# avi22bhattacharya/ThinkDiff-mlre

Hardware: AMD Instinct MI355X
Metric: images/sec (1024², 28 steps) ThinkDiff-CLIP FLUX.1 at 1/2/4/8 MI355X (higher is better)
Workload: dtype bf16

## Files before the change

thinkdiff-mlre_amd/csrc/attention_bf16.hip:

```cpp
#include "attention_common.h"

template <bool CAUSAL, int NWAVES, bool BIAS = false, bool VARLEN = false, bool PRE = false, bool RS = true, bool FIXED = false>
__global__ __launch_bounds__(NWAVES * 64, 2) void td_attn_fwd_d128_lean_kernel(const TdAttnParams p) {
#if defined(__HIP_DEVICE_COMPILE__)
  extern __shared__ __attribute__((aligned(16))) char smem[];

  const int tid = threadIdx.x;
  const int lane = tid & 63;
  const int wid = __builtin_amdgcn_readfirstlane(tid >> 6);
  const int h5 = lane >> 5;
  const int l31 = lane & 31;

  const int qblk = blockIdx.x;
  const int head = blockIdx.y;
  const int batch = blockIdx.z;
  const int kvhead = head / p.q_per_kv;
  const int q0 = qblk * (NWAVES * Q_WAVE) + wid * Q_WAVE;

  const bf16_t* Qb = p.Q + (size_t)batch * p.q_bstride;
  const bf16_t* Kb = p.K + (size_t)batch * p.kv_bstride;
  const bf16_t* Vb = p.V + (size_t)batch * p.kv_bstride;
  bf16_t* Ob = p.O + (size_t)batch * p.o_bstride;
  int Sq = p.Sq, Skv = p.Skv, c_off = p.causal_offset;
  if constexpr (VARLEN) {
// ... 276 lines not shown

      f32x16_t st[2];
      attn_tile_scores<PO, FIXED>(st, qf, kone, qnegm, ka);

      const int key0 = t * KV_TILE;
      if (key0 + KV_TILE > Skv) {
#pragma unroll
        for (int kk = 0; kk < 2; ++kk)
#pragma unroll
          for (int rr = 0; rr < 16; ++rr) {
            const int key = key0 + kk * 32 + (rr & 3) + 8 * (rr >> 2) + 4 * h5;
            if (key >= Skv) st[kk][rr] = -INFINITY;
          }
      }

      attn_tile_softmax_pv<PO, PRE, RS, FIXED>(st, o, lacc, m_run, qnegm, t == kb, c, va, h5);
    };
    {
      int t = kb;
      for (; t + 1 < ke; t += 2) {
        tile(t, std::integral_constant<unsigned, 0>{});
        tile(t + 1, std::integral_constant<unsigned, 1>{});
      }
      if (t < ke) tile(t, std::integral_constant<unsigned, 0>{});
    }
    float l_run = RS ? lacc[0] : half_swap_sum(lacc[0]);
    if (kb > 0 || ke < nt) {
      const int j = kb > 0 ? r : r + 1;
      const bool tail = kb > 0;
      const __amdgpu_buffer_rsrc_t rsS = __builtin_amdgcn_make_buffer_rsrc((void*)(ws + SK_HEADER_BYTES), 0, (unsigned)(2 * G) * SK_SLOT_FLOATS * 4u, 0x00020000);
      const unsigned lane_off = ((unsigned)wid * 17u * 64u + (unsigned)lane) * 16u;
      const unsigned mine = (unsigned)(tail ? j : G + j) * (SK_SLOT_FLOATS * 4u) + lane_off;
      const unsigned theirs = (unsigned)(tail ? G + j : j) * (SK_SLOT_FLOATS * 4u) + lane_off;
      auto ask = [&](bool draw) -> unsigned {
        __syncthreads();
        if (tid == 0)
          *ticket_lds = draw ? __hip_atomic_fetch_add(cnt + j, 1u, __ATOMIC_RELAXED, __HIP_MEMORY_SCOPE_AGENT)
                             : __hip_atomic_load(cnt + j, __ATOMIC_RELAXED, __HIP_MEMORY_SCOPE_AGENT);
        __syncthreads();
        return *ticket_lds;
      };
      bool other_ready = !tail && ask(false) == 1u;
      if (!other_ready) {
#pragma unroll
        for (int q4 = 0; q4 < 16; ++q4) {
          const u32x4_t v = {as_u32(o[q4 >> 2][4 * (q4 & 3)]), as_u32(o[q4 >> 2][4 * (q4 & 3) + 1]),
                             as_u32(o[q4 >> 2][4 * (q4 & 3) + 2]), as_u32(o[q4 >> 2][4 * (q4 & 3) + 3])};
          __builtin_amdgcn_raw_buffer_store_b128(v, rsS, mine + q4 * 1024u, 0, 16);
        }
        const u32x4_t ml = {as_u32(m_run), as_u32(l_run), 0u, 0u};
        __builtin_amdgcn_raw_buffer_store_b128(ml, rsS, mine + 16 * 1024u, 0, 16);
        asm volatile("s_waitcnt vmcnt(0)" ::: "memory");
        other_ready = ask(true) == 1u;
        if (!other_ready) continue;
      }
      if (tid == 0) __builtin_amdgcn_fence(__ATOMIC_ACQUIRE, "agent");
      asm volatile("s_waitcnt vmcnt(0)" ::: "memory");
      __syncthreads();
      const u32x4_t ml = __builtin_amdgcn_raw_buffer_load_b128(rsS, theirs + 16 * 1024u, 0, 0);
      const float m2 = as_f32(ml[0]), l2 = as_f32(ml[1]);
      const float mm = fmaxf(m_run, m2);
      const float a1 = __builtin_amdgcn_exp2f((m_run - mm) * cc), a2 = __builtin_amdgcn_exp2f((m2 - mm) * cc);
      auto comb = [&](float own, float other) {
        return tail ? __builtin_fmaf(other, a2, own * a1) : __builtin_fmaf(own, a1, other * a2);
      };
      l_run = comb(l_run, l2);
#pragma unroll
      for (int q4 = 0; q4 < 16; ++q4) {
        const u32x4_t v = __builtin_amdgcn_raw_buffer_load_b128(rsS, theirs + q4 * 1024u, 0, 0);
#pragma unroll
        for (int k4 = 0; k4 < 4; ++k4)
          o[q4 >> 2][4 * (q4 & 3) + k4] = comb(o[q4 >> 2][4 * (q4 & 3) + k4], as_f32(v[k4]));
      }
      if (tid == 0) __hip_atomic_store(cnt + j, 0u, __ATOMIC_RELAXED, __HIP_MEMORY_SCOPE_AGENT);
    }

    const float inv = 1.0f / l_run;
    const int q = q0 + l31;
    if (p.q8) {
      const int qr = min(q, p.Sq - 1);
      attn_store_rows_q8(o, inv, p.q8 + (size_t)qr * p.ldq8 + head * D, h5, p.q8_inv[qr], p.q8_amax + qr, q < p.Sq);
    } else {
      attn_store_rows(o, inv, p.O + (size_t)batch * p.o_bstride + (size_t)min(q, p.Sq - 1) * p.ldo + head * D, h5, (p.ldo & 7) == 0 && !(p.variant & 0x200), q < p.Sq);
    }
  }
#endif
}

namespace {

size_t sk_ws_bytes(int ranges) { return (size_t)SK_HEADER_BYTES + (size_t)2 * ranges * SK_SLOT_FLOATS * sizeof(float); }

int sk_pooled_workspace(int dev, int ranges, hipStream_t stream, char** out) {
  struct Entry { int dev; hipStream_t stream; int ranges; char* ws; };
  static std::mutex mu;
  static std::vector<Entry> pool;
  std::lock_guard<std::mutex> lock(mu);
  for (auto& e : pool)
    if (e.dev == dev && e.stream == stream && e.ranges >= ranges) { *out = e.ws; return 0; }
  char* w = nullptr;
  TD_CHECK_HIP(hipMalloc((void**)&w, sk_ws_bytes(ranges)));
  TD_CHECK_HIP(hipMemsetAsync(w, 0, SK_HEADER_BYTES, stream));
  pool.push_back(Entry{dev, stream, ranges, w});
  *out = w;
  return 0;
}

int device_cus(int dev) {
  static std::atomic<int> cus[64] = {};
  int n = cus[dev & 63].load(std::memory_order_relaxed);
  if (n == 0) {
    hipDeviceProp_t prop;
    if (hipGetDeviceProperties(&prop, dev) != hipSuccess) return 0;
    n = prop.multiProcessorCount;
    cus[dev & 63].store(n, std::memory_order_relaxed);
  }
  return n;
}

template <typename K>
int set_lds_attr_once(K kernel, int bytes, std::atomic<unsigned long long>& done, int dev) {
  if (!((done.load(std::memory_order_acquire) >> (dev & 63)) & 1ull)) {
    TD_CHECK_HIP(hipFuncSetAttribute((const void*)kernel, hipFuncAttributeMaxDynamicSharedMemorySize, bytes));
    done.fetch_or(1ull << (dev & 63), std::memory_order_release);
  }
  return 0;
}

}

int td_attn_device_cus(int dev) { return device_cus(dev); }
int td_attn_pooled_workspace(int dev, int ranges, hipStream_t stream, char** out) { return sk_pooled_workspace(dev, ranges, stream, out); }
int td_attn_set_lds_attr(const void* kernel, int bytes, std::atomic<unsigned long long>& done, int dev) {
  if (!((done.load(std::memory_order_acquire) >> (dev & 63)) & 1ull)) {
    TD_CHECK_HIP(hipFuncSetAttribute(kernel, hipFuncAttributeMaxDynamicSharedMemorySize, bytes));
    done.fetch_or(1ull << (dev & 63), std::memory_order_release);
  }
  return 0;
}

int td_attn_launch(const TdAttnParams& p, hipStream_t stream) {
  TD_CHECK_ARG(p.head_dim == D, "td_attention: head_dim=%d unsupported (only 128)", p.head_dim);
  TD_CHECK_ARG(p.Sq > 0 && p.Skv > 0 && p.Hq > 0 && p.Hkv > 0 && p.batch > 0, "td_attention: empty problem");
  TD_CHECK_ARG(p.Hq % p.Hkv == 0, "td_attention: Hq=%d not a multiple of Hkv=%d", p.Hq, p.Hkv);
  TD_CHECK_ARG(p.ldq % 8 == 0 && p.ldkv % 8 == 0 && p.ldo % 4 == 0, "td_attention: row strides must be 16-byte multiples");
  TD_CHECK_ARG(((long long)(p.Sq + 256) * p.ldq) * 2 < (1ll << 32) && ((long long)(p.Skv + 64) * p.ldkv) * 2 < (1ll << 32),
               "td_attention: per-batch operand exceeds the 4 GiB buffer-descriptor range");
  TD_CHECK_ARG(((uintptr_t)p.Q | (uintptr_t)p.K | (uintptr_t)p.V | (uintptr_t)p.O) % 16 == 0, "td_attention: pointers must be 16-byte aligned");
  if (p.Sq == 1 && p.causal && !p.bias && (p.variant & 0xff) == 0 && (p.kv_lens || p.causal_offset == p.Skv - 1))
    return td_attn_decode_launch(p, stream);
  TdAttnParams q = p;
  q.q_per_kv = p.Hq / p.Hkv;
  constexpr int NW = 8;
  constexpr int lds = 4 * TILE_BYTES;
  int dev = 0;
  TD_CHECK_HIP(hipGetDevice(&dev));
  static std::atomic<unsigned long long> a0{0}, a1{0}, a2{0}, a3{0}, a4{0}, a5{0};
  dim3 grid((p.Sq + NW * Q_WAVE - 1) / (NW * Q_WAVE), p.Hq, p.batch);
  if (p.bias) TD_CHECK_ARG(p.Skv % 4 == 0 && ((uintptr_t)p.bias) % 16 == 0 && p.batch == 1, "td_attention: bias needs Skv %% 4 == 0, 16-byte alignment, batch 1");
  if (p.kv_lens) TD_CHECK_ARG(p.causal && !p.bias, "td_attention: per-sequence kv lengths exist for the causal kernel only");
  if (p.q_prescaled) TD_CHECK_ARG(!p.causal && !p.bias && !p.kv_lens && !p.seg_starts, "td_attention: pre-scaled q is a form of the joint (unmasked) attention only");
  TD_CHECK_ARG(p.score_bound >= 0.f && p.score_bound <= 48.f && (p.score_bound == 0.f || p.q_prescaled), "td_attention: a score bound goes with pre-scaled q (joint attention) and lies in (0, 48] octaves (0 = none)");
  if (p.q8) TD_CHECK_ARG(!p.causal && !p.bias && !p.kv_lens && !p.seg_starts && p.batch == 1 && p.q8_inv && p.q8_amax && p.ldq8 % 8 == 0 && ((uintptr_t)p.q8) % 8 == 0,
                         "td_attention: the int8 output form is for the joint attention of one batch entry, with 8-byte aligned rows");
  if (p.seg_starts) {
    TD_CHECK_ARG(!p.bias && !p.kv_lens && p.Sq == p.Skv && (!p.causal || p.causal_offset == 0),
                 "td_attention(varlen): full or causal (offset 0) attention inside each segment only (no bias or cache lengths)");
    if (p.causal) {
      static std::atomic<unsigned long long> a12{0};
      if (int e = set_lds_attr_once(td_attn_fwd_d128_lean_kernel<true, NW, false, true>, lds, a12, dev)) return e;
      hipLaunchKernelGGL((td_attn_fwd_d128_lean_kernel<true, NW, false, true>), grid, dim3(NW * 64), lds, stream, q);
      TD_CHECK_LAUNCH();
      return 0;
    }
    static std::atomic<unsigned long long> a6{0};
    if (int e = set_lds_attr_once(td_attn_fwd_d128_lean_kernel<false, NW, false, true>, lds, a6, dev)) return e;
    hipLaunchKernelGGL((td_attn_fwd_d128_lean_kernel<false, NW, false, true>), grid, dim3(NW * 64), lds, stream, q);
    TD_CHECK_LAUNCH();
    return 0;
  }

  const int n_items = (int)(grid.x * grid.y * grid.z);
  const int cus = device_cus(dev);
  const int nt = (p.Skv + KV_TILE - 1) / KV_TILE;
  if (!p.causal && !p.bias && !p.kv_lens && (p.variant & 0xff) != 1 && cus > 0 && n_items > cus && cus < SK_MAX_RANGES && (long long)n_items * nt < (1ll << 31)) {
    char* ws = (char*)p.sk_ws;
    if (!ws) {
      if (int rc = sk_pooled_workspace(dev, cus, stream, &ws)) return rc;
    }
    constexpr int lds_sk = lds + 16;
    if (p.q_prescaled && p.score_bound > 0.f) {
      static std::atomic<unsigned long long> a10{0};
      if (int e = set_lds_attr_once(td_attn_fwd_d128_streamk_kernel<NW, true, true, true, true>, lds_sk, a10, dev)) return e;
      hipLaunchKernelGGL((td_attn_fwd_d128_streamk_kernel<NW, true, true, true, true>), dim3(cus), dim3(NW * 64), lds_sk, stream, q, ws, (int)grid.x, nt);
    } else if (p.q_prescaled) {
      static std::atomic<unsigned long long> a7{0};
      if (int e = set_lds_attr_once(td_attn_fwd_d128_streamk_kernel<NW, true, true>, lds_sk, a7, dev)) return e;
      hipLaunchKernelGGL((td_attn_fwd_d128_streamk_kernel<NW, true, true>), dim3(cus), dim3(NW * 64), lds_sk, stream, q, ws, (int)grid.x, nt);
    } else if ((p.variant & 0xff) == 2) {
      if (int e = set_lds_attr_once(td_attn_fwd_d128_streamk_kernel<NW, false>, lds_sk, a4, dev)) return e;
      hipLaunchKernelGGL((td_attn_fwd_d128_streamk_kernel<NW, false>), dim3(cus), dim3(NW * 64), lds_sk, stream, q, ws, (int)grid.x, nt);
    } else {
      if (int e = set_lds_attr_once(td_attn_fwd_d128_streamk_kernel<NW, true>, lds_sk, a5, dev)) return e;
      hipLaunchKernelGGL((td_attn_fwd_d128_streamk_kernel<NW, true>), dim3(cus), dim3(NW * 64), lds_sk, stream, q, ws, (int)grid.x, nt);
    }
    TD_CHECK_LAUNCH();
    return 0;
  }
  if (p.bias) {
    if (p.causal) {
      if (int e = set_lds_attr_once(td_attn_fwd_d128_lean_kernel<true, NW, true>, lds, a0, dev)) return e;
      hipLaunchKernelGGL((td_attn_fwd_d128_lean_kernel<true, NW, true>), grid, dim3(NW * 64), lds, stream, q);
    } else {
      if (int e = set_lds_attr_once(td_attn_fwd_d128_lean_kernel<false, NW, true>, lds, a1, dev)) return e;
      hipLaunchKernelGGL((td_attn_fwd_d128_lean_kernel<false, NW, true>), grid, dim3(NW * 64), lds, stream, q);
    }
  } else {
    if (p.q_prescaled && p.score_bound > 0.f) {
      static std::atomic<unsigned long long> a11{0};
      if (int e = set_lds_attr_once(td_attn_fwd_d128_lean_kernel<false, NW, false, false, true, true, true>, lds, a11, dev)) return e;
      hipLaunchKernelGGL((td_attn_fwd_d128_lean_kernel<false, NW, false, false, true, true, true>), grid, dim3(NW * 64), lds, stream, q);
    } else if (p.q_prescaled) {
      static std::atomic<unsigned long long> a8{0};
      if (int e = set_lds_attr_once(td_attn_fwd_d128_lean_kernel<false, NW, false, false, true>, lds, a8, dev)) return e;
      hipLaunchKernelGGL((td_attn_fwd_d128_lean_kernel<false, NW, false, false, true>), grid, dim3(NW * 64), lds, stream, q);
    } else if (p.causal) {
      if (int e = set_lds_attr_once(td_attn_fwd_d128_lean_kernel<true, NW>, lds, a2, dev)) return e;
      hipLaunchKernelGGL((td_attn_fwd_d128_lean_kernel<true, NW>), grid, dim3(NW * 64), lds, stream, q);
    } else {
      if (int e = set_lds_attr_once(td_attn_fwd_d128_lean_kernel<false, NW>, lds, a3, dev)) return e;
      hipLaunchKernelGGL((td_attn_fwd_d128_lean_kernel<false, NW>), grid, dim3(NW * 64), lds, stream, q);
    }
  }
  TD_CHECK_LAUNCH();
  return 0;
}

size_t td_attn_streamk_ws_bytes() {
  int dev = 0;
  if (hipGetDevice(&dev) != hipSuccess) return 0;
  const int cus = device_cus(dev);
  return cus > 0 && cus < SK_MAX_RANGES ? sk_ws_bytes(cus) : 0;
}
```

thinkdiff-mlre_amd/csrc/attention_common.h:

```cpp
#pragma once
#include <atomic>
#include <mutex>
#include <type_traits>
#include <vector>

#include "td_common.h"
#include "td_kernels.h"

namespace {

constexpr int D = 128;
constexpr int KV_TILE = 64;
constexpr int Q_WAVE = 32;
constexpr int TILE_BYTES = KV_TILE * D * 2;

__device__ __forceinline__ void half_swap(float x, float& lo, float& hi) {
  lo = x;
  hi = x;
  asm volatile("s_nop 1\n\tv_permlane32_swap_b32 %0, %1\n\ts_nop 1" : "+v"(lo), "+v"(hi));
}
__device__ __forceinline__ float max3(float a, float b, float c) {
  float r;
  asm("v_max3_f32 %0, %1, %2, %3" : "=v"(r) : "v"(a), "v"(b), "v"(c));
  return r;
// ... 104 lines not shown
      }
      pf[kb][s] = __builtin_bit_cast(bf16x8_t, pk);
    }
  }
  if constexpr (!RS) lacc[0] += psum;

  constexpr int VPF = 2;
  const bf16x8_t ones8 = {0x3F80, 0x3F80, 0x3F80, 0x3F80, 0x3F80, 0x3F80, 0x3F80, 0x3F80};
  bf16x4_t v0[16], v1[16];
  attn_static_for<VPF>([&](auto ec) {
    constexpr int e = decltype(ec)::value;
    v0[e] = attn_ds_read_tr16<PO + (e >> 2) * 16 * 256>(va[0][e & 3]);
    v1[e] = attn_ds_read_tr16<PO + (e >> 2) * 16 * 256>(va[1][e & 3]);
  });
  attn_static_for<16>([&](auto ec) {
    constexpr int e = decltype(ec)::value;
    if constexpr (e + VPF < 16) {
      v0[e + VPF] = attn_ds_read_tr16<PO + ((e + VPF) >> 2) * 16 * 256>(va[0][(e + VPF) & 3]);
      v1[e + VPF] = attn_ds_read_tr16<PO + ((e + VPF) >> 2) * 16 * 256>(va[1][(e + VPF) & 3]);
    }
    constexpr int behind = 2 * (15 - e < VPF ? 15 - e : VPF);
    asm volatile("s_waitcnt lgkmcnt(%2)" : "+v"(v0[e]), "+v"(v1[e]) : "n"(behind));
    bf16x8_t vf;
    vf[0] = v0[e][0]; vf[1] = v0[e][1]; vf[2] = v0[e][2]; vf[3] = v0[e][3];
    vf[4] = v1[e][0]; vf[5] = v1[e][1]; vf[6] = v1[e][2]; vf[7] = v1[e][3];
    o[e & 3] = __builtin_amdgcn_mfma_f32_32x32x16_bf16(vf, pf[e >> 3][(e >> 2) & 1], o[e & 3], 0, 0, 0);
    if constexpr (RS && (e & 3) == 3) lacc = __builtin_amdgcn_mfma_f32_32x32x16_bf16(ones8, pf[e >> 3][(e >> 2) & 1], lacc, 0, 0, 0);
    __builtin_amdgcn_sched_barrier(0x006);
  });
}

__device__ __forceinline__ void attn_store_rows(const f32x16_t (&o)[4], const float inv, bf16_t* row_ptr, const int h5, const bool wide, const bool live) {
  if (wide) {
#pragma unroll
    for (int db = 0; db < 4; ++db)
#pragma unroll
      for (int g = 0; g < 4; g += 2) {
        unsigned a0 = pack_bf2(o[db][4 * g] * inv, o[db][4 * g + 1] * inv), a1 = pack_bf2(o[db][4 * g + 2] * inv, o[db][4 * g + 3] * inv);
        unsigned b0 = pack_bf2(o[db][4 * g + 4] * inv, o[db][4 * g + 5] * inv), b1 = pack_bf2(o[db][4 * g + 6] * inv, o[db][4 * g + 7] * inv);
        const auto r0 = __builtin_amdgcn_permlane32_swap(a0, b0, false, false);
        const auto r1 = __builtin_amdgcn_permlane32_swap(a1, b1, false, false);
        const u32x4_t w = {r0[0], r1[0], r0[1], r1[1]};
        if (live) *(u32x4_t*)(row_ptr + db * 32 + 8 * (g + h5)) = w;
      }
  } else {
#pragma unroll
    for (int db = 0; db < 4; ++db)
#pragma unroll
      for (int g = 0; g < 4; ++g) {
        u32x2_t w;
        w[0] = pack_bf2(o[db][4 * g] * inv, o[db][4 * g + 1] * inv);
        w[1] = pack_bf2(o[db][4 * g + 2] * inv, o[db][4 * g + 3] * inv);
        if (live) *(u32x2_t*)(row_ptr + 4 * h5 + db * 32 + 8 * g) = w;
      }
  }
}

__device__ __forceinline__ void attn_store_rows_q8(const f32x16_t (&o)[4], const float inv, uint8_t* row_ptr, const int h5, const float qinv, unsigned* amax,
                                                   const bool live) {
  float am = 0.f;
#pragma unroll
  for (int db = 0; db < 4; ++db)
#pragma unroll
    for (int g = 0; g < 4; g += 2) {
      unsigned w[2];
#pragma unroll
      for (int h = 0; h < 2; ++h) {
        unsigned acc = 0;
#pragma unroll
        for (int b = 0; b < 4; ++b) {
          const float v = rbf(o[db][4 * (g + h) + b] * inv);
          am = fmaxf(am, fabsf(v));
          acc |= ((unsigned)__float2int_rn(fminf(fmaxf(v * qinv, -127.f), 127.f)) & 0xffu) << (8 * b);
        }
        w[h] = acc;
      }
      const auto r = __builtin_amdgcn_permlane32_swap(w[0], w[1], false, false);
      if (live) *(u32x2_t*)(row_ptr + db * 32 + 8 * (g + h5)) = u32x2_t{r[0], r[1]};
    }
  am = half_swap_max(am);
  if (live && h5 == 0) __hip_atomic_fetch_max(amax, as_u32(am), __ATOMIC_RELAXED, __HIP_MEMORY_SCOPE_AGENT);
}

}

int td_attn_set_lds_attr(const void* kernel, int bytes, std::atomic<unsigned long long>& done, int dev);

namespace {
constexpr int SK_SLOT_FLOATS = 8 * 64 * 68;
constexpr int SK_HEADER_BYTES = 4096;
constexpr int SK_MAX_RANGES = SK_HEADER_BYTES / 4 - 16;
}
```

thinkdiff-mlre_amd/csrc/capi.hip:

```cpp
#include <cstdarg>
#include <cstdio>
#include "td_kernels.h"
#include "../../include/thinkdiff_hip.h"

static thread_local char g_err[512] = "";

void td_set_error(const char* fmt, ...) {
  va_list ap;
  va_start(ap, fmt);
  vsnprintf(g_err, sizeof(g_err), fmt, ap);
  va_end(ap);
}

extern "C" {

const char* td_last_error(void) { return g_err; }
int td_abi_version(void) { return 1; }

int td_linear_bf16(const void* x, int64_t ldx, const void* w, const void* bias, void* y, int64_t ldy,
                   int M, int N, int K, int act, const void* gate, const void* res, int64_t ldr,
                   void* stream) {
  TdGemmParams p;
  p.A = (const bf16_t*)x; p.lda = (int)ldx;
  p.W = (const bf16_t*)w; p.bias = (const bf16_t*)bias;
// ... 3 lines not shown
  return td_gemm_launch(p, (hipStream_t)stream);
}

int td_linear_split_bf16(const void* x, int64_t ldx, const void* w, const void* bias,
                         void* y0, int64_t ldy0, int act0, void* y1, int64_t ldy1, int act1,
                         int M, int N, int K, int n_split, void* stream) {
  TdGemmParams p;
  p.A = (const bf16_t*)x; p.lda = (int)ldx;
  p.W = (const bf16_t*)w; p.bias = (const bf16_t*)bias;
  p.C = (bf16_t*)y0; p.ldc = (int)ldy0; p.act = act0;
  p.C2 = (bf16_t*)y1; p.ldc2 = (int)ldy1; p.act2 = act1; p.n_split = n_split;
  p.M = M; p.N = N; p.K = K;
  return td_gemm_launch(p, (hipStream_t)stream);
}

int td_linear_splitk_bf16(const void* x, int64_t ldx, const void* w, const void* bias, void* y0, int64_t ldy0, void* y1, int64_t ldy1, int n_split,
                          int M, int N, int K, const void* res, int64_t ldr, int tile_cfg, int split_k,
                          const void* norm_w, void* norm_out, int64_t ld_norm, float norm_eps, void* stream) {
  TdGemmParams p;
  p.sk_norm_w = (const bf16_t*)norm_w; p.sk_norm_out = (bf16_t*)norm_out; p.sk_norm_ld = (int)ld_norm; p.sk_norm_eps = norm_eps;
  p.A = (const bf16_t*)x; p.lda = (int)ldx; p.W = (const bf16_t*)w; p.bias = (const bf16_t*)bias;
  p.C = (bf16_t*)y0; p.ldc = (int)ldy0; p.C2 = (bf16_t*)y1; p.ldc2 = (int)ldy1; p.n_split = y1 ? n_split : 0;
  p.res = (const bf16_t*)res; p.ldr = (int)ldr; p.M = M; p.N = N; p.K = K; p.cfg = tile_cfg; p.split_k = split_k;
  return td_gemm_launch(p, (hipStream_t)stream);
}

int td_linear_grouped2_bf16(const void* x0, int M0, const void* w0, const void* bias0, const void* gate0,
                            const void* res0, void* y0, const void* x1, int M1, const void* w1,
                            const void* bias1, const void* gate1, const void* res1, void* y1,
                            int64_t ldx, int64_t ldy, int64_t ldr, int N, int K, int act, int tile_cfg,
                            void* stream) {
  TdGemmParams p;
  p.A = (const bf16_t*)x0; p.W = (const bf16_t*)w0; p.bias = (const bf16_t*)bias0; p.gate = (const bf16_t*)gate0;
  p.res = (const bf16_t*)res0; p.C = (bf16_t*)y0; p.M = M0;
  p.g_A = (const bf16_t*)x1; p.g_W = (const bf16_t*)w1; p.g_bias = (const bf16_t*)bias1; p.g_gate = (const bf16_t*)gate1;
  p.g_res = (const bf16_t*)res1; p.g_C = (bf16_t*)y1; p.g_M = M1;
  p.lda = (int)ldx; p.ldc = (int)ldy; p.ldr = (int)ldr; p.N = N; p.K = K; p.act = act; p.cfg = tile_cfg;
  return td_gemm_launch(p, (hipStream_t)stream);
}

int td_conv3x3_nhwc_bf16(const void* x, const void* w, const void* bias, const void* res, void* y,
                         int H, int W, int Cin, int Cout, int upsample2x, void* stream) {
  TdGemmParams p;
  p.A = (const bf16_t*)x; p.lda = Cin; p.W = (const bf16_t*)w; p.bias = (const bf16_t*)bias;
  p.C = (bf16_t*)y; p.ldc = Cout; p.res = (const bf16_t*)res; p.ldr = Cout;
  p.M = H * W; p.N = Cout; p.K = 9 * Cin;
  p.conv_H = H; p.conv_W = W; p.conv_Cin = Cin; p.conv_up = upsample2x ? 1 : 0;
  return td_gemm_launch(p, (hipStream_t)stream);
}

int td_linear_f32out_bf16(const void* x, int64_t ldx, const void* w, const void* bias, float* y, int64_t ldy,
                          int M, int N, int K, void* stream) {
  TdGemmParams p;
  p.A = (const bf16_t*)x; p.lda = (int)ldx; p.W = (const bf16_t*)w; p.bias = (const bf16_t*)bias;
  p.C = (bf16_t*)y; p.ldc = (int)ldy; p.M = M; p.N = N; p.K = K; p.out_f32 = 1; p.cfg = (N <= 64) ? 1 : (M <= 32 ? 2 : 0);
  return td_gemm_launch(p, (hipStream_t)stream);
}

static int g_attn_variant = 0;
int td_attention_set_variant(int variant) {
  const int prev = g_attn_variant;
  g_attn_variant = variant;
  return prev;
}

int td_attention_bf16(const void* q, int64_t ldq, int64_t q_bstride, const void* k, const void* v,
                      int64_t ldkv, int64_t kv_bstride, void* o, int64_t ldo, int64_t o_bstride,
                      int batch, int Sq, int Skv, int Hq, int Hkv, int head_dim, float scale,
                      int causal, void* stream) {
  TdAttnParams p;
  p.Q = (const bf16_t*)q; p.K = (const bf16_t*)k; p.V = (const bf16_t*)v; p.O = (bf16_t*)o;
  p.batch = batch; p.Sq = Sq; p.Skv = Skv; p.Hq = Hq; p.Hkv = Hkv; p.head_dim = head_dim;
  p.ldq = (int)ldq; p.ldkv = (int)ldkv; p.ldo = (int)ldo;
  p.q_bstride = q_bstride; p.kv_bstride = kv_bstride; p.o_bstride = o_bstride;
  p.scale = scale; p.causal = causal; p.causal_offset = Skv - Sq; p.variant = g_attn_variant & ~0x800;
  p.q_prescaled = (g_attn_variant & 0x800) && !causal ? 1 : 0;
  return td_attn_launch(p, (hipStream_t)stream);
}

int td_attention_joint_prescaled_bf16(const void* q, int64_t ldq, const void* k, const void* v, int64_t ldkv, void* o, int64_t ldo, int S, int H, float score_bound, void* stream) {
  TdAttnParams p;
  p.Q = (const bf16_t*)q; p.K = (const bf16_t*)k; p.V = (const bf16_t*)v; p.O = (bf16_t*)o;
  p.batch = 1; p.Sq = S; p.Skv = S; p.Hq = H; p.Hkv = H; p.head_dim = 128;
  p.ldq = (int)ldq; p.ldkv = (int)ldkv; p.ldo = (int)ldo; p.scale = 1.0f; p.causal = 0; p.causal_offset = 0; p.variant = g_attn_variant & 0xff;
  p.q_prescaled = 1; p.score_bound = score_bound;
  return td_attn_launch(p, (hipStream_t)stream);
}

size_t td_attention_fp8_workspace_bytes(int Sq, int Skv, int Hq) { return Sq > 0 && Skv > 0 && Hq > 0 ? td_attn_fp8_ws_bytes(Sq, Skv, Hq) : 0; }

int td_attention_fp8(const void* q, int64_t ldq, const void* k, const void* v, int64_t ldkv, void* o, int64_t ldo,
                     int Sq, int Skv, int Hq, float scale, void* workspace, void* stream) {
  TdAttnParams p;
  p.Q = (const bf16_t*)q; p.K = (const bf16_t*)k; p.V = (const bf16_t*)v; p.O = (bf16_t*)o;
  p.batch = 1; p.Sq = Sq; p.Skv = Skv; p.Hq = Hq; p.Hkv = Hq; p.head_dim = 128;
  p.ldq = (int)ldq; p.ldkv = (int)ldkv; p.ldo = (int)ldo; p.scale = scale; p.f8_ws = workspace; p.variant = ((g_attn_variant & 1) ? 0x1000 : 0) | ((g_attn_variant & 2) ? 0x2000 : 0) | (((g_attn_variant >> 4) & 7) << 16);
  return td_attn_fp8_launch(p, (hipStream_t)stream);
}

int td_attention_fp8_qk_rope(const void* qkv, int64_t ld, int q_col, int k_col, int v_col, void* o, int64_t ldo, int S, int H,
                             const float* cos, const float* sin, int split, const void* wqA, const void* wkA, const void* wqB, const void* wkB,
                             float eps, float scale, void* workspace, void* stream) {
  TD_CHECK_ARG(qkv && cos && sin && q_col >= 0 && k_col >= 0 && v_col >= 0 && (q_col | k_col | v_col) % 8 == 0, "td_attention_fp8_qk_rope: projection buffer, both tables, 16-byte aligned column offsets");
  TD_CHECK_ARG(S > 0 && H > 0 && (long long)(q_col > k_col ? (q_col > v_col ? q_col : v_col) : (k_col > v_col ? k_col : v_col)) + (long long)H * 128 <= ld,
               "td_attention_fp8_qk_rope: the q / k / v head blocks (H=%d x 128 columns from their offsets) do not fit a row of ld=%lld", H, (long long)ld);
  TdAttnParams p;
  p.Q = (const bf16_t*)qkv + q_col; p.K = (const bf16_t*)qkv + k_col; p.V = (const bf16_t*)qkv + v_col; p.O = (bf16_t*)o;
  p.batch = 1; p.Sq = S; p.Skv = S; p.Hq = H; p.Hkv = H; p.head_dim = 128;
  p.ldq = (int)ld; p.ldkv = (int)ld; p.ldo = (int)ldo; p.scale = scale; p.f8_ws = workspace; p.variant = ((g_attn_variant & 1) ? 0x1000 : 0) | ((g_attn_variant & 2) ? 0x2000 : 0);
  p.rope_cos = cos; p.rope_sin = sin; p.rope_split = split; p.rope_eps = eps;
  p.rope_wqA = (const bf16_t*)wqA; p.rope_wkA = (const bf16_t*)wkA; p.rope_wqB = (const bf16_t*)wqB; p.rope_wkB = (const bf16_t*)wkB;
  return td_attn_fp8_launch(p, (hipStream_t)stream);
}

int td_attention_varlen_bf16(const void* q, int64_t ldq, const void* k, const void* v, int64_t ldkv, void* o, int64_t ldo,
                             const int* seg_starts, int n_seg, int max_len, int Hq, int Hkv, float scale, void* stream) {
  TD_CHECK_ARG(seg_starts && n_seg > 0 && max_len > 0, "td_attention_varlen: empty segment list");
  TdAttnParams p;
  p.Q = (const bf16_t*)q; p.K = (const bf16_t*)k; p.V = (const bf16_t*)v; p.O = (bf16_t*)o;
  p.batch = n_seg; p.Sq = max_len; p.Skv = max_len; p.Hq = Hq; p.Hkv = Hkv; p.head_dim = 128;
  p.ldq = (int)ldq; p.ldkv = (int)ldkv; p.ldo = (int)ldo;
  p.scale = scale; p.causal = 0; p.causal_offset = 0; p.variant = 1; p.seg_starts = seg_starts;
  return td_attn_launch(p, (hipStream_t)stream);
}

int td_norm_rows_bf16(const void* x, int64_t ldx, void* y, int64_t ldy, int rows, int D, int rms, float eps,
                      const void* w, int split, const void* shiftA, const void* scaleA,
                      const void* shiftB, const void* scaleB, void* stream) {
  TdNormParams p;
  p.x = (const bf16_t*)x; p.ldx = (int)ldx; p.y = (bf16_t*)y; p.ldy = (int)ldy; p.rows = rows; p.D = D;
  p.rms = rms; p.eps = eps; p.w = (const bf16_t*)w; p.split = split;
  p.shiftA = (const bf16_t*)shiftA; p.scaleA = (const bf16_t*)scaleA;
  p.shiftB = (const bf16_t*)shiftB; p.scaleB = (const bf16_t*)scaleB;
  if (p.scaleA && !p.scaleB) { p.scaleB = p.scaleA; p.shiftB = p.shiftA; }
  return td_norm_rows_launch(p, (hipStream_t)stream);
}

int td_qk_norm_rope_bf16(void* qkv, int64_t ld, int rows, int Hq, int Hk, int q_col, int k_col,
                         const float* cos, const float* sin, int split, const void* wqA, const void* wkA,
                         const void* wqB, const void* wkB, float eps, int rotate_half, void* stream) {
  TdQkRopeParams p;
  p.qkv = (bf16_t*)qkv; p.ld = (int)ld; p.rows = rows; p.Hq = Hq; p.Hk = Hk; p.q_col = q_col; p.k_col = k_col;
  p.cos = cos; p.sin = sin; p.split = split;
  p.wqA = (const bf16_t*)wqA; p.wkA = (const bf16_t*)wkA; p.wqB = (const bf16_t*)wqB; p.wkB = (const bf16_t*)wkB;
  p.eps = eps; p.rotate_half = rotate_half;
  return td_qk_norm_rope_launch(p, (hipStream_t)stream);
}

int td_flux_rope_table(const float* ids, int S, const int* axes_dims3, double theta, float* cos, float* sin, void* stream) {
  return td_flux_rope_table_launch(ids, S, axes_dims3, theta, cos, sin, (hipStream_t)stream);
}
int td_timestep_sincos(const float* t, int n, void* out, void* stream) {
  return td_timestep_sincos_launch(t, n, (bf16_t*)out, (hipStream_t)stream);
}
int td_euler_step_bf16(void* x, const void* v, float dt, int64_t n, void* stream) {
  return td_euler_step_launch((bf16_t*)x, (const bf16_t*)v, dt, n, (hipStream_t)stream);
}
int td_flux_pack_latents(const void* src, void* dst, int C, int H, int W, int unpack, float div, float add, void* stream) {
  return td_flux_pack_launch((const bf16_t*)src, (bf16_t*)dst, C, H, W, unpack, div, add, (hipStream_t)stream);
}
int td_cls_avgpool2_bf16(const void* x, void* y, int G, int C, void* stream) {
  return td_cls_avgpool2_launch((const bf16_t*)x, (bf16_t*)y, G, C, (hipStream_t)stream);
}

int td_aligner_mlp2x_bf16(const void* x, int64_t ldx, int M, int K, int hidden, const void* w0, const void* b0,
                          const void* w2, const void* b2, const void* norm_w, float eps, int fp32_norm,
                          void* workspace, void* y, int64_t ldy, void* stream) {
// ... 127 lines not shown
```

Measured before the change: 0.6063.

## Add fixed-max 16x16 MFMA attention kernel for prescaled bounded joint attention

Adds a new attention kernel for the prescaled, score-bounded, non-causal path. It uses 16x16x32 bf16 MFMA tiles and skips the online running max, since a known score bound allows a fixed exp2 with no rescaling. The row sum is accumulated by an MFMA against a ones vector. A stream-K variant merges partial results through a workspace by plain addition, and dispatch routes eligible calls to it, with variant bit 0x400 as an opt-out. This is meant to remove max tracking and rescale work and to improve MFMA shape use, at the risk of overflow if the score bound is wrong.

```diff
diff --git a/thinkdiff-mlre_amd/csrc/attention_bf16.hip b/thinkdiff-mlre_amd/csrc/attention_bf16.hip
--- a/thinkdiff-mlre_amd/csrc/attention_bf16.hip
+++ b/thinkdiff-mlre_amd/csrc/attention_bf16.hip
@@ -382,6 +382,198 @@
       attn_store_rows_q8(o, inv, p.q8 + (size_t)qr * p.ldq8 + head * D, h5, p.q8_inv[qr], p.q8_amax + qr, q < p.Sq);
     } else {
       attn_store_rows(o, inv, p.O + (size_t)batch * p.o_bstride + (size_t)min(q, p.Sq - 1) * p.ldo + head * D, h5, (p.ldo & 7) == 0 && !(p.variant & 0x200), q < p.Sq);
+    }
+  }
+#endif
+}
+
+template <int NWAVES, bool STREAMK>
+__global__ __launch_bounds__(NWAVES * 64, 2) void td_attn_fwd_d128_fixed16_kernel(const TdAttnParams p, char* __restrict__ ws,
+                                                                                  const int n_qblk, const int nt) {
+#if defined(__HIP_DEVICE_COMPILE__)
+  extern __shared__ __attribute__((aligned(16))) char smem[];
+  const int tid = threadIdx.x;
+  const int lane = tid & 63;
+  const int wid = __builtin_amdgcn_readfirstlane(tid >> 6);
+  const int g = lane >> 4;
+  const int l15 = lane & 15;
+
+  long long it, it_end;
+  int r = 0;
+  if constexpr (STREAMK) {
+    const int G = gridDim.x;
+    r = blockIdx.x;
+    const int q8 = G >> 3, r8 = G & 7, xcd = r & 7;
+    r = (xcd < r8 ? xcd * (q8 + 1) : r8 * (q8 + 1) + (xcd - r8) * q8) + (r >> 3);
+    const long long total = (long long)n_qblk * p.Hq * p.batch * nt;
+    it = total * r / G;
+    it_end = total * (r + 1) / G;
+  } else {
+    it = ((long long)(blockIdx.z * p.Hq + blockIdx.y) * n_qblk + blockIdx.x) * nt;
+    it_end = it + nt;
+  }
+
+  const int Skv = p.Skv;
+  constexpr int GROUPS = KV_TILE / 4;
+  constexpr int SG = (GROUPS + NWAVES - 1) / NWAVES;
+  const int srow = lane >> 4;
+
+  const unsigned lds0 = (unsigned)(uintptr_t)(TD_LDS char*)smem;
+  unsigned ka[4];
+  {
+    const unsigned kr = attn16_key(l15);
+    const unsigned ksw = ((kr & 3) << 2) | ((kr >> 2) & 3);
+#pragma unroll
+    for (int ks = 0; ks < 4; ++ks) ka[ks] = lds0 + kr * 256 + (((4 * ks + g) ^ ksw) << 4);
+  }
+  unsigned va[8];
+  {
+    const unsigned vq = (lane & 15) >> 2, vp = lane & 3;
+    const unsigned vr = attn16_key(4 * g + vq);
+    const unsigned swz = ((vr & 3) << 2) | ((vr >> 2) & 3);
+#pragma unroll
+    for (int db = 0; db < 8; ++db) va[db] = lds0 + 2 * TILE_BYTES + vr * 256 + (((2 * db + (vp >> 1)) ^ swz) << 4) + 8 * (vp & 1);
+  }
+
+  if ((p.variant & 0x100) && wid >= 4) __builtin_amdgcn_s_setprio(1);
+  while (it < it_end) {
+    const int item = (int)(it / nt);
+    const int kb = (int)(it - (long long)item * nt);
+    const int ke = (int)min((long long)nt, kb + (it_end - it));
+    __builtin_assume(ke > kb);
+    it += ke - kb;
+    const int qblk = item % n_qblk;
+    const int hb = item / n_qblk;
+    const int head = hb % p.Hq, batch = hb / p.Hq;
+    const int kvhead = head / p.q_per_kv;
+    const int q0 = qblk * (NWAVES * Q_WAVE) + wid * Q_WAVE;
+
+    const bf16_t* Qb = p.Q + (size_t)batch * p.q_bstride;
+    const bf16_t* Kb = p.K + (size_t)batch * p.kv_bstride;
+    const bf16_t* Vb = p.V + (size_t)batch * p.kv_bstride;
+    const unsigned q_bytes = (unsigned)(((long long)(p.Sq - 1) * p.ldq + p.Hq * D) * 2);
+    const unsigned kv_bytes = (unsigned)(((long long)(Skv - 1) * p.ldkv + p.Hkv * D) * 2);
+    __amdgpu_buffer_rsrc_t rsQ = __builtin_amdgcn_make_buffer_rsrc((void*)Qb, 0, q_bytes, 0x00020000);
+    __amdgpu_buffer_rsrc_t rsK = __builtin_amdgcn_make_buffer_rsrc((void*)Kb, 0, kv_bytes, 0x00020000);
+    __amdgpu_buffer_rsrc_t rsV = __builtin_amdgcn_make_buffer_rsrc((void*)Vb, 0, kv_bytes, 0x00020000);
+
+    unsigned voffK[SG];
+#pragma unroll
+    for (int s = 0; s < SG; ++s) {
+      const int gg = wid + NWAVES * s;
+      const int swz = (srow << 2) | (gg & 3);
+      const int chunk = (lane & 15) ^ swz;
+      voffK[s] = (unsigned)(gg * 4 + srow) * (unsigned)p.ldkv * 2u + (unsigned)(kvhead * D + chunk * 8) * 2u;
+    }
+    auto stage = [&](int slot, int t) {
+      const unsigned tile_off = (unsigned)t * KV_TILE * (unsigned)p.ldkv * 2u;
+#pragma unroll
+      for (int s = 0; s < SG; ++s) {
+        const int gg = wid + NWAVES * s;
+        if (GROUPS % NWAVES == 0 || gg < GROUPS) {
+          __builtin_amdgcn_raw_ptr_buffer_load_lds(rsK, (TD_LDS void*)(smem + slot * TILE_BYTES + gg * 1024), 16, voffK[s] + tile_off, 0, 0, 0);
+          __builtin_amdgcn_raw_ptr_buffer_load_lds(rsV, (TD_LDS void*)(smem + (2 + slot) * TILE_BYTES + gg * 1024), 16, voffK[s] + tile_off, 0, 0, 0);
+        }
+      }
+    };
+    if constexpr (STREAMK) __syncthreads();
+    stage(0, kb);
+
+    bf16x8_t qf[2][4];
+#pragma unroll
+    for (int qb = 0; qb < 2; ++qb) {
+      const unsigned qoff = (unsigned)(q0 + 16 * qb + l15) * (unsigned)p.ldq * 2u + (unsigned)(head * D + 8 * g) * 2u;
+#pragma unroll
+      for (int ks = 0; ks < 4; ++ks) qf[qb][ks] = __builtin_bit_cast(bf16x8_t, __builtin_amdgcn_raw_buffer_load_b128(rsQ, qoff + ks * 64, 0, 0));
+    }
+
+    f32x4_t o[8][2], lacc[2];
+#pragma unroll
+    for (int qb = 0; qb < 2; ++qb) {
+#pragma unroll
+      for (int db = 0; db < 8; ++db) o[db][qb] = f32x4_t{0.f, 0.f, 0.f, 0.f};
+      lacc[qb] = f32x4_t{0.f, 0.f, 0.f, 0.f};
+    }
+    auto tile = [&](const int t, auto slot_tag) {
+      constexpr unsigned SLOT = decltype(slot_tag)::value;
+      constexpr unsigned PO = SLOT * TILE_BYTES;
+      asm volatile("s_waitcnt vmcnt(0)" ::: "memory");
+      __syncthreads();
+      if (t + 1 < ke) stage(SLOT ^ 1, t + 1);
+
+      f32x4_t st[4][2];
+      attn16_tile_scores<PO>(st, qf, ka);
+
+      const int key0 = t * KV_TILE;
+      if (key0 + KV_TILE > Skv) {
+#pragma unroll
+        for (int kb4 = 0; kb4 < 4; ++kb4)
+#pragma unroll
+          for (int rr = 0; rr < 4; ++rr) {
+            const int key = key0 + 16 * kb4 + attn16_key(4 * g + rr);
+            if (key >= Skv) { st[kb4][0][rr] = -INFINITY; st[kb4][1][rr] = -INFINITY; }
+          }
+      }
+      attn16_tile_softmax_pv<PO>(st, o, lacc, va);
+    };
+    {
+      int t = kb;
+      for (; t + 1 < ke; t += 2) {
+        tile(t, std::integral_constant<unsigned, 0>{});
+        tile(t + 1, std::integral_constant<unsigned, 1>{});
+      }
+      if (t < ke) tile(t, std::integral_constant<unsigned, 0>{});
+    }
+    float l_run[2] = {lacc[0][0], lacc[1][0]};
+
+    if constexpr (STREAMK) {
+      if (kb > 0 || ke < nt) {
+        const int G = gridDim.x;
+        unsigned* const cnt = (unsigned*)ws + 16;
+        TD_LDS unsigned* const ticket_lds = (TD_LDS unsigned*)(smem + 4 * TILE_BYTES);
+        const int j = kb > 0 ? r : r + 1;
+        const bool tail = kb > 0;
+        const __amdgpu_buffer_rsrc_t rsS = __builtin_amdgcn_make_buffer_rsrc((void*)(ws + SK_HEADER_BYTES), 0, (unsigned)(2 * G) * SK_SLOT_FLOATS * 4u, 0x00020000);
+        const unsigned lane_off = ((unsigned)wid * 17u * 64u + (unsigned)lane) * 16u;
+        const unsigned mine = (unsigned)(tail ? j : G + j) * (SK_SLOT_FLOATS * 4u) + lane_off;
+        const unsigned theirs = (unsigned)(tail ? G + j : j) * (SK_SLOT_FLOATS * 4u) + lane_off;
+        auto ask = [&](bool draw) -> unsigned {
+          __syncthreads();
+          if (tid == 0)
+            *ticket_lds = draw ? __hip_atomic_fetch_add(cnt + j, 1u, __ATOMIC_RELAXED, __HIP_MEMORY_SCOPE_AGENT)
+                               : __hip_atomic_load(cnt + j, __ATOMIC_RELAXED, __HIP_MEMORY_SCOPE_AGENT);
+          __syncthreads();
+          return *ticket_lds;
+        };
+        bool other_ready = !tail && ask(false) == 1u;
+        if (!other_ready) {
+#pragma unroll
+          for (int c4 = 0; c4 < 16; ++c4)
+            __builtin_amdgcn_raw_buffer_store_b128(__builtin_bit_cast(u32x4_t, o[c4 >> 1][c4 & 1]), rsS, mine + c4 * 1024u, 0, 16);
+          const u32x4_t ll = {as_u32(l_run[0]), as_u32(l_run[1]), 0u, 0u};
+          __builtin_amdgcn_raw_buffer_store_b128(ll, rsS, mine + 16 * 1024u, 0, 16);
+          asm volatile("s_waitcnt vmcnt(0)" ::: "memory");
+          other_ready = ask(true) == 1u;
+          if (!other_ready) continue;
+        }
+        if (tid == 0) __builtin_amdgcn_fence(__ATOMIC_ACQUIRE, "agent");
+        asm volatile("s_waitcnt vmcnt(0)" ::: "memory");
+        __syncthreads();
+        const u32x4_t ll = __builtin_amdgcn_raw_buffer_load_b128(rsS, theirs + 16 * 1024u, 0, 0);
+        l_run[0] += as_f32(ll[0]);
+        l_run[1] += as_f32(ll[1]);
+#pragma unroll
+        for (int c4 = 0; c4 < 16; ++c4)
+          o[c4 >> 1][c4 & 1] += __builtin_bit_cast(f32x4_t, __builtin_amdgcn_raw_buffer_load_b128(rsS, theirs + c4 * 1024u, 0, 0));
+        if (tid == 0) __hip_atomic_store(cnt + j, 0u, __ATOMIC_RELAXED, __HIP_MEMORY_SCOPE_AGENT);
+      }
+    }
+
+    const bool wide = (p.ldo & 7) == 0 && !(p.variant & 0x200);
+#pragma unroll
+    for (int qb = 0; qb < 2; ++qb) {
+      const int q = q0 + 16 * qb + l15;
+      attn16_store_rows(o, qb, 1.0f / l_run[qb], p.O + (size_t)batch * p.o_bstride + (size_t)min(q, p.Sq - 1) * p.ldo + head * D, g, wide, q < p.Sq);
     }
   }
 #endif
@@ -483,13 +675,18 @@
   const int n_items = (int)(grid.x * grid.y * grid.z);
   const int cus = device_cus(dev);
   const int nt = (p.Skv + KV_TILE - 1) / KV_TILE;
+  const bool fixed16 = p.q_prescaled && p.score_bound > 0.f && !p.causal && !p.bias && !p.kv_lens && !p.q8 && !(p.variant & 0x400);
   if (!p.causal && !p.bias && !p.kv_lens && (p.variant & 0xff) != 1 && cus > 0 && n_items > cus && cus < SK_MAX_RANGES && (long long)n_items * nt < (1ll << 31)) {
     char* ws = (char*)p.sk_ws;
     if (!ws) {
       if (int rc = sk_pooled_workspace(dev, cus, stream, &ws)) return rc;
     }
     constexpr int lds_sk = lds + 16;
-    if (p.q_prescaled && p.score_bound > 0.f) {
+    if (fixed16) {
+      static std::atomic<unsigned long long> a13{0};
+      if (int e = set_lds_attr_once(td_attn_fwd_d128_fixed16_kernel<NW, true>, lds_sk, a13, dev)) return e;
+      hipLaunchKernelGGL((td_attn_fwd_d128_fixed16_kernel<NW, true>), dim3(cus), dim3(NW * 64), lds_sk, stream, q, ws, (int)grid.x, nt);
+    } else if (p.q_prescaled && p.score_bound > 0.f) {
       static std::atomic<unsigned long long> a10{0};
       if (int e = set_lds_attr_once(td_attn_fwd_d128_streamk_kernel<NW, true, true, true, true>, lds_sk, a10, dev)) return e;
       hipLaunchKernelGGL((td_attn_fwd_d128_streamk_kernel<NW, true, true, true, true>), dim3(cus), dim3(NW * 64), lds_sk, stream, q, ws, (int)grid.x, nt);
@@ -516,7 +713,11 @@
       hipLaunchKernelGGL((td_attn_fwd_d128_lean_kernel<false, NW, true>), grid, dim3(NW * 64), lds, stream, q);
     }
   } else {
-    if (p.q_prescaled && p.score_bound > 0.f) {
+    if (fixed16) {
+      static std::atomic<unsigned long long> a14{0};
+      if (int e = set_lds_attr_once(td_attn_fwd_d128_fixed16_kernel<NW, false>, lds, a14, dev)) return e;
+      hipLaunchKernelGGL((td_attn_fwd_d128_fixed16_kernel<NW, false>), grid, dim3(NW * 64), lds, stream, q, (char*)nullptr, (int)grid.x, nt);
+    } else if (p.q_prescaled && p.score_bound > 0.f) {
       static std::atomic<unsigned long long> a11{0};
       if (int e = set_lds_attr_once(td_attn_fwd_d128_lean_kernel<false, NW, false, false, true, true, true>, lds, a11, dev)) return e;
       hipLaunchKernelGGL((td_attn_fwd_d128_lean_kernel<false, NW, false, false, true, true, true>), grid, dim3(NW * 64), lds, stream, q);
diff --git a/thinkdiff-mlre_amd/csrc/attention_common.h b/thinkdiff-mlre_amd/csrc/attention_common.h
--- a/thinkdiff-mlre_amd/csrc/attention_common.h
+++ b/thinkdiff-mlre_amd/csrc/attention_common.h
@@ -210,6 +210,95 @@
   if (live && h5 == 0) __hip_atomic_fetch_max(amax, as_u32(am), __ATOMIC_RELAXED, __HIP_MEMORY_SCOPE_AGENT);
 }
 
+__device__ __forceinline__ constexpr int attn16_key(const int i) { return 8 * ((i >> 2) & 1) + 4 * (i >> 3) + (i & 3); }
+
+template <unsigned PO>
+__device__ __forceinline__ void attn16_tile_scores(f32x4_t (&st)[4][2], const bf16x8_t (&qf)[2][4], const unsigned (&ka)[4]) {
+  constexpr int KPF = 2;
+  const f32x4_t zero4 = {0.f, 0.f, 0.f, 0.f};
+  auto kread = [&](int e) {
+    return *(const TD_LDS bf16x8_t*)(uintptr_t)(ka[e & 3] + PO + (e >> 2) * 16 * 256);
+  };
+  bf16x8_t kf[16];
+#pragma unroll
+  for (int e = 0; e < KPF; ++e) kf[e] = kread(e);
+  __builtin_amdgcn_sched_group_barrier(0x100, KPF, 0);
+#pragma unroll
+  for (int e = 0; e < 16; ++e) {
+    if (e + KPF < 16) kf[e + KPF] = kread(e + KPF);
+#pragma unroll
+    for (int qb = 0; qb < 2; ++qb)
+      st[e >> 2][qb] = __builtin_amdgcn_mfma_f32_16x16x32_bf16(kf[e], qf[qb][e & 3], (e & 3) == 0 ? zero4 : st[e >> 2][qb], 0, 0, 0);
+    if (e + KPF < 16) __builtin_amdgcn_sched_group_barrier(0x100, 1, 0);
+    __builtin_amdgcn_sched_group_barrier(0x008, 2, 0);
+  }
+}
+
+template <unsigned PO>
+__device__ __forceinline__ void attn16_tile_softmax_pv(const f32x4_t (&st)[4][2], f32x4_t (&o)[8][2], f32x4_t (&lacc)[2], const unsigned (&va)[8]) {
+  bf16x8_t pf[2][2];
+#pragma unroll
+  for (int s = 0; s < 2; ++s)
+#pragma unroll
+    for (int qb = 0; qb < 2; ++qb) {
+      u32x4_t pk;
+#pragma unroll
+      for (int h = 0; h < 2; ++h)
+#pragma unroll
+        for (int j = 0; j < 2; ++j)
+          pk[2 * h + j] = pack_bf2(__builtin_amdgcn_exp2f(st[2 * s + h][qb][2 * j]), __builtin_amdgcn_exp2f(st[2 * s + h][qb][2 * j + 1]));
+      pf[s][qb] = __builtin_bit_cast(bf16x8_t, pk);
+    }
+  constexpr int VPF = 2;
+  const bf16x8_t ones8 = {0x3F80, 0x3F80, 0x3F80, 0x3F80, 0x3F80, 0x3F80, 0x3F80, 0x3F80};
+  bf16x4_t v0[16], v1[16];
+  attn_static_for<VPF>([&](auto ec) {
+    constexpr int e = decltype(ec)::value;
+    v0[e] = attn_ds_read_tr16<PO + (2 * (e >> 3)) * 16 * 256>(va[e & 7]);
+    v1[e] = attn_ds_read_tr16<PO + (2 * (e >> 3) + 1) * 16 * 256>(va[e & 7]);
+  });
+  attn_static_for<16>([&](auto ec) {
+    constexpr int e = decltype(ec)::value;
+    if constexpr (e + VPF < 16) {
+      v0[e + VPF] = attn_ds_read_tr16<PO + (2 * ((e + VPF) >> 3)) * 16 * 256>(va[(e + VPF) & 7]);
+      v1[e + VPF] = attn_ds_read_tr16<PO + (2 * ((e + VPF) >> 3) + 1) * 16 * 256>(va[(e + VPF) & 7]);
+    }
+    constexpr int behind = 2 * (15 - e < VPF ? 15 - e : VPF);
+    asm volatile("s_waitcnt lgkmcnt(%2)" : "+v"(v0[e]), "+v"(v1[e]) : "n"(behind));
+    bf16x8_t vf;
+    vf[0] = v0[e][0]; vf[1] = v0[e][1]; vf[2] = v0[e][2]; vf[3] = v0[e][3];
+    vf[4] = v1[e][0]; vf[5] = v1[e][1]; vf[6] = v1[e][2]; vf[7] = v1[e][3];
+#pragma unroll
+    for (int qb = 0; qb < 2; ++qb) o[e & 7][qb] = __builtin_amdgcn_mfma_f32_16x16x32_bf16(vf, pf[e >> 3][qb], o[e & 7][qb], 0, 0, 0);
+    if constexpr ((e & 7) == 7) {
+#pragma unroll
+      for (int qb = 0; qb < 2; ++qb) lacc[qb] = __builtin_amdgcn_mfma_f32_16x16x32_bf16(ones8, pf[e >> 3][qb], lacc[qb], 0, 0, 0);
+    }
+    __builtin_amdgcn_sched_barrier(0x006);
+  });
+}
+
+__device__ __forceinline__ void attn16_store_rows(const f32x4_t (&o)[8][2], const int qb, const float inv, bf16_t* row_ptr, const int g, const bool wide,
+                                                  const bool live) {
+  if (wide) {
+#pragma unroll
+    for (int m = 0; m < 4; ++m) {
+      const unsigned a0 = pack_bf2(o[2 * m][qb][0] * inv, o[2 * m][qb][1] * inv), a1 = pack_bf2(o[2 * m][qb][2] * inv, o[2 * m][qb][3] * inv);
+      const unsigned b0 = pack_bf2(o[2 * m + 1][qb][0] * inv, o[2 * m + 1][qb][1] * inv), b1 = pack_bf2(o[2 * m + 1][qb][2] * inv, o[2 * m + 1][qb][3] * inv);
+      const auto r0 = __builtin_amdgcn_permlane16_swap(a0, b0, false, false);
+      const auto r1 = __builtin_amdgcn_permlane16_swap(a1, b1, false, false);
+      const u32x4_t w = {r0[0], r1[0], r0[1], r1[1]};
+      if (live) *(u32x4_t*)(row_ptr + 16 * (2 * m + (g & 1)) + 8 * (g >> 1)) = w;
+    }
+  } else {
+#pragma unroll
+    for (int db = 0; db < 8; ++db) {
+      const u32x2_t w = {pack_bf2(o[db][qb][0] * inv, o[db][qb][1] * inv), pack_bf2(o[db][qb][2] * inv, o[db][qb][3] * inv)};
+      if (live) *(u32x2_t*)(row_ptr + 16 * db + 4 * g) = w;
+    }
+  }
+}
+
 }
 
 int td_attn_set_lds_attr(const void* kernel, int bytes, std::atomic<unsigned long long>& done, int dev);
diff --git a/thinkdiff-mlre_amd/csrc/capi.hip b/thinkdiff-mlre_amd/csrc/capi.hip
--- a/thinkdiff-mlre_amd/csrc/capi.hip
+++ b/thinkdiff-mlre_amd/csrc/capi.hip
@@ -109,7 +109,8 @@
   TdAttnParams p;
   p.Q = (const bf16_t*)q; p.K = (const bf16_t*)k; p.V = (const bf16_t*)v; p.O = (bf16_t*)o;
   p.batch = 1; p.Sq = S; p.Skv = S; p.Hq = H; p.Hkv = H; p.head_dim = 128;
-  p.ldq = (int)ldq; p.ldkv = (int)ldkv; p.ldo = (int)ldo; p.scale = 1.0f; p.causal = 0; p.causal_offset = 0; p.variant = g_attn_variant & 0xff;
+  p.ldq = (int)ldq; p.ldkv = (int)ldkv; p.ldo = (int)ldo; p.scale = 1.0f; p.causal = 0; p.causal_offset = 0;
+  p.variant = g_attn_variant & 0x4ff;
   p.q_prescaled = 1; p.score_bound = score_bound;
   return td_attn_launch(p, (hipStream_t)stream);
 }
```

New measurement: 0.6138 (median of 6 runs). 1.01x the previous value.
